# BuTTerK3ks/AA-RMVSNet

Measured on AMD Instinct MI355X. Metric: depth-hypotheses/sec (ref-views x H x W x D / s), higher is better.
Workload: dtype fp32-class split-fp16 (3 products: cells, deconvs, omega conv on f16 MFMA, lo*lo dropped, fp32 accumulate; fp32 elsewhere); 1 GPU; dtu_eval_1600x1184_n7_d512; ref_views_per_gpu=1, views=7, H=1184, W=1600, D=512, global_batch=1, parallelism=ref-view shard x1

## Files before the change

aa-rmvsnet_amd/csrc/convlstm.hip:

```cpp
#include <hip/hip_runtime.h>

#include <cstdlib>
#include <cstring>

#include <algorithm>
#include <type_traits>

#include "device_common.h"

namespace aarmvs {

typedef float floatx16 __attribute__((ext_vector_type(16)));

enum SrcMode : int { SRC_PLAIN = 0, SRC_POOL = 1, SRC_GNRELU = 2 };

struct ChanSrc {
  const float* ptr;
  int nch;
  int mode;
  const double* stats;
  const float* gamma;
  const float* beta;
  const double* part;
  int nblk;
  double* stats_out;
};

__device__ __forceinline__ void gn_table(const ChanSrc& s, float* gn, double* red, int tid, int H, int W) {
  if (!s.part) {
    if (tid < 16) {
      const GnStat st = stat_read(s.stats + (tid >> 3) * kSlots * 2, 8.0 * H * W);
      const float sc = st.rstd * s.gamma[tid];
      gn[tid] = sc;
      gn[16 + tid] = s.beta[tid] - st.mean * sc;
    }
    return;
  }
  if (tid < 256) {
    double acc[4] = {0.0, 0.0, 0.0, 0.0};
    for (int i = tid; i < s.nblk; i += 256)
#pragma unroll
      for (int j = 0; j < 4; ++j) acc[j] += s.part[4 * i + j];
#pragma unroll
    for (int j = 0; j < 4; ++j) red[j * 256 + tid] = acc[j];
  }
  __syncthreads();
  for (int o = 128; o > 0; o >>= 1) {
    if (tid < o)
#pragma unroll
      for (int j = 0; j < 4; ++j) red[j * 256 + tid] += red[j * 256 + tid + o];
    __syncthreads();
  }
  if (tid < 16) {
    const int g = tid >> 3;
    const GnStat st = gn_stat_from(red[2 * g * 256], red[(2 * g + 1) * 256], 8.0 * H * W);
    const float sc = st.rstd * s.gamma[tid];
    gn[tid] = sc;
    gn[16 + tid] = s.beta[tid] - st.mean * sc;
  }
  if (blockIdx.x == 0 && tid < 4) s.stats_out[(tid >> 1) * kSlots * 2 + (tid & 1)] = red[tid * 256];
  __syncthreads();
}

struct CellArgs {
  ChanSrc part[3];
  int nparts;
  float* h_new;
  float* c;
  const float* c_in;
  float* z_out;
  const float* wpk;
  const float* bias;
  const unsigned* xbound;
  int B, H, W;
  int skew;
};

constexpr int kHScaleExp = 12;

__device__ __forceinline__ int guard_exp_of(float bound) {
  if (!(bound > 0.0f)) return 0;
  const int k = ilogbf(bound);
  return k >= 134 ? 120 : (k < -100 ? -114 : k - 14);
}
__device__ __forceinline__ int xguard_exp(const unsigned* xb) {
  return xb ? guard_exp_of(__uint_as_float(*xb)) : -kHScaleExp;
}
__device__ __forceinline__ int gguard_exp(const float* gamma, const float* beta, int H, int W) {
  return guard_exp_of(gn_relu_bound(gamma, beta, 8.0 * H * W));
}

constexpr int kMaxParts = 3;

template <int KIND>
struct CellDef;
#ifndef AARMVS_C3DB
#define AARMVS_C3DB 1
#endif
#ifndef AARMVS_C4DB
#define AARMVS_C4DB 0
#endif
#ifndef AARMVS_C3SKEW
#define AARMVS_C3SKEW 3
#endif
#ifndef AARMVS_C4SKEW
#define AARMVS_C4SKEW 0
#endif
#ifndef AARMVS_C4PIPE
#define AARMVS_C4PIPE 0
#endif
template <>
struct CellDef<0> {
  static constexpr int NP = 2, CH[kMaxParts] = {32, 16, 0};
  static constexpr int MODE[kMaxParts] = {SRC_PLAIN, SRC_PLAIN, SRC_PLAIN};
  static constexpr int HID = 16;
  static constexpr int H3RW = 1, H3WAVES = 8, H3DB = 1, H3PIPE = 1, H3MS = 1;
  static constexpr int MIN_WAVES = 1;
  static constexpr int SKEW = 3;
};
template <>
struct CellDef<1> {
  static constexpr int NP = 2, CH[kMaxParts] = {16, 16, 0};
  static constexpr int MODE[kMaxParts] = {SRC_POOL, SRC_PLAIN, SRC_PLAIN};
  static constexpr int HID = 16;
  static constexpr int H3RW = 1, H3WAVES = 8, H3DB = 1, H3PIPE = 1, H3MS = 1;
  static constexpr int MIN_WAVES = 1;
  static constexpr int SKEW = 2;
};
template <>
struct CellDef<2> : CellDef<1> {};
template <>
struct CellDef<3> {
  static constexpr int NP = 3, CH[kMaxParts] = {16, 16, 16};
  static constexpr int MODE[kMaxParts] = {SRC_GNRELU, SRC_PLAIN, SRC_PLAIN};
  static constexpr int HID = 16;
  static constexpr int H3RW = 1, H3WAVES = 8, H3DB = AARMVS_C3DB, H3PIPE = 1, H3MS = 1;
  static constexpr int MIN_WAVES = 1;
  static constexpr int SKEW = AARMVS_C3SKEW;
};
template <>
struct CellDef<4> {
  static constexpr int NP = 3, CH[kMaxParts] = {16, 16, 8};
  static constexpr int MODE[kMaxParts] = {SRC_GNRELU, SRC_PLAIN, SRC_PLAIN};
  static constexpr int HID = 8;
  static constexpr int H3RW = 1, H3WAVES = 8, H3DB = AARMVS_C4DB, H3PIPE = AARMVS_C4PIPE, H3MS = 1;
  static constexpr int MIN_WAVES = 4;
  static constexpr int SKEW = AARMVS_C4SKEW;
};

typedef _Float16 half8 __attribute__((ext_vector_type(8)));
typedef _Float16 half2_t __attribute__((ext_vector_type(2)));

template <int KIND, int RW_ = CellDef<KIND>::H3RW, int WAVES_ = CellDef<KIND>::H3WAVES, int MS_ = 1>
struct H3Cfg {
  using D = CellDef<KIND>;
  static constexpr int CIN = D::CH[0] + D::CH[1] + D::CH[2];
  static constexpr int NCHK = (CIN + 15) / 16;
  static constexpr int HID = D::HID, MT = HID / 8, COUT = 4 * HID;
  static constexpr int RW = RW_, WAVES = WAVES_, MS = MS_, MTL = MT / MS, RWAVES = WAVES / MS;
  static_assert(MT % MS == 0 && WAVES % MS == 0, "whole m-tiles and rows per wave");
  static constexpr int TH = RW * RWAVES, THREADS = WAVES * 64, TW = 32, W2 = TW + 2, TROWS = TH + 2;
  static constexpr int NPIX = TROWS * W2;
  static constexpr int A_HALVES = NCHK * 9 * MT * 64 * 8;
  static constexpr size_t LDS_BYTES = (size_t)A_HALVES * 2 * 2 + (size_t)NPIX * 32 * 2 + 32 * 4;
  static constexpr int c0(int p) { return p == 0 ? 0 : (p == 1 ? D::CH[0] : D::CH[0] + D::CH[1]); }
  static constexpr int chunk_part(int c) {
    return 16 * c < c0(1) ? 0 : (16 * c < c0(2) || D::NP < 3 ? 1 : 2);
  }
  static constexpr int chunk_lc0(int c) { return 16 * c - c0(chunk_part(c)); }
  static constexpr int chunk_nv(int c) {
    return D::CH[chunk_part(c)] - chunk_lc0(c) < 16 ? D::CH[chunk_part(c)] - chunk_lc0(c) : 16;
  }
  static constexpr bool chunk_paired(int c) { return chunk_nv(c) == 8; }
};

__device__ __forceinline__ int h3_pix(int p, int h) { return p * 32 + ((h ^ ((p >> 3) & 1)) << 4); }

typedef float float2_t __attribute__((ext_vector_type(2)));
__device__ __forceinline__ uint32_t h3_split2(float a, float b, uint32_t& lo_bits) {
  const half2_t hi = __builtin_convertvector((float2_t){a, b}, half2_t);
  const half2_t lo = __builtin_convertvector((float2_t){a - (float)hi[0], b - (float)hi[1]}, half2_t);
  lo_bits = __builtin_bit_cast(uint32_t, lo);
  return __builtin_bit_cast(uint32_t, hi);
}

template <int KIND, int RW, int WAVES, int NTH = 0, bool PAIRSKIP = false, int MS = 1>
struct H3PixStager {
  using C = H3Cfg<KIND, RW, WAVES, MS>;
  using D = typename C::D;
  static constexpr int TH = NTH ? NTH : C::THREADS;
  static constexpr int NITEM = 2 * C::NPIX;
  static constexpr int NI = (NITEM + TH - 1) / TH;
  static_assert(NI <= 32, "item mask holds 32 items");
  float val[NI][8][4];
  uint32_t in_mask;
  float xs = 1.0f;

  template <int CH>
  __device__ __forceinline__ void load(const CellArgs& a, int b, int y0, int x0, int tid) {
    constexpr int P = C::chunk_part(CH), MODE = D::MODE[P], NCH = D::CH[P];
    constexpr int LC0 = C::chunk_lc0(CH), NV = C::chunk_nv(CH);
    static_assert(NV % 8 == 0, "chunks hold whole 8-channel halves");
    const ChanSrc& s = a.part[P];
    const int H = a.H, W = a.W;
    const int Hs = MODE == SRC_POOL ? 2 * H : H, Ws = MODE == SRC_POOL ? 2 * W : W;
    const uint32_t nbytes = (uint32_t)NCH * (uint32_t)Hs * (uint32_t)Ws * 4u;
    const __amdgpu_buffer_rsrc_t r = uniform_rsrc(s.ptr + (size_t)b * NCH * Hs * Ws, nbytes);
    in_mask = 0u;
#pragma unroll
    for (int j = 0; j < NI; ++j) {
      const int e = tid + j * TH;
      const int h = e >= C::NPIX ? 1 : 0, p = e - h * C::NPIX;
      if (PAIRSKIP && C::chunk_paired(CH) && h) continue;
      const int row = p / C::W2, col = p - row * C::W2;
      const int gy = y0 - 1 + row, gx = x0 - 1 + col;
      const bool in = e < NITEM && 8 * h < NV && gy >= 0 && gy < H && gx >= 0 && gx < W;
      if (in) in_mask |= 1u << j;
      const uint32_t pix = MODE == SRC_POOL ? (uint32_t)(2 * gy * Ws + 2 * gx) : (uint32_t)(gy * W + gx);
      const uint32_t ob = (pix * (uint32_t)NCH + (uint32_t)(LC0 + 8 * h)) * 4u;
      constexpr int NW = MODE == SRC_POOL ? 4 : 1;
#pragma unroll
      for (int w = 0; w < NW; ++w) {
        const uint32_t o = in ? ob + (uint32_t)(((w >> 1) * Ws + (w & 1)) * NCH * 4) : nbytes;
        const float4 q0 = ld4(r, o), q1 = ld4(r, in ? o + 16u : nbytes);
        val[j][0][w] = q0.x;
        val[j][1][w] = q0.y;
        val[j][2][w] = q0.z;
        val[j][3][w] = q0.w;
        val[j][4][w] = q1.x;
        val[j][5][w] = q1.y;
        val[j][6][w] = q1.z;
        val[j][7][w] = q1.w;
      }
    }
  }

  template <int CH>
  __device__ __forceinline__ void store(char* hi_plane, char* lo_plane, const float* gn, int tid,
                                        int x0, int W) const {
    constexpr int MODE = D::MODE[C::chunk_part(CH)];
    constexpr int LC0 = C::chunk_lc0(CH);
#pragma unroll
    for (int j = 0; j < NI; ++j) {
      const int e = tid + j * TH;
      if (e < NITEM) {
        const int h = e >= C::NPIX ? 1 : 0, p = e - h * C::NPIX;
        if (PAIRSKIP && C::chunk_paired(CH) && h) continue;
        const bool in = in_mask & (1u << j);
        float v[8];
#pragma unroll
        for (int k = 0; k < 8; ++k) {
          float x;
          constexpr float HS = (float)(1 << kHScaleExp);
          if (MODE == SRC_POOL) {
            x = fmaxf(fmaxf(val[j][k][0], val[j][k][1]), fmaxf(val[j][k][2], val[j][k][3])) * HS;
          } else if (MODE == SRC_GNRELU) {
            const int lc = LC0 + 8 * h + k;
            x = fmaxf(val[j][k][0] * gn[lc] + gn[16 + lc], 0.0f) * xs;
          } else if constexpr (KIND == 0 && C::chunk_part(CH) == 0) {
            x = val[j][k][0] * xs;
          } else {
            x = val[j][k][0] * HS;
          }
          v[k] = in ? x : 0.0f;
        }
        uint32_t hw[4], lw[4];
#pragma unroll
        for (int i = 0; i < 4; ++i) hw[i] = h3_split2(v[2 * i], v[2 * i + 1], lw[i]);
        const int off = h3_pix(p, h);
        *reinterpret_cast<u32x4*>(hi_plane + off) = u32x4{hw[0], hw[1], hw[2], hw[3]};
        *reinterpret_cast<u32x4*>(lo_plane + off) = u32x4{lw[0], lw[1], lw[2], lw[3]};
      }
    }
  }
};

template <class C, int KIND, int CH, bool BAL>
__device__ __forceinline__ void xguard_rescale(floatx16 (&acc)[C::MTL][C::RW], floatx16 (&accn)[C::MTL][C::RW],
                                               float xr) {
  if constexpr ((KIND == 0 || C::D::MODE[0] == SRC_GNRELU) && CH > 0 && C::chunk_part(CH) != 0 &&
                C::chunk_part(CH - 1) == 0) {
#pragma unroll
    for (int m = 0; m < C::MTL; ++m)
#pragma unroll
      for (int r = 0; r < C::RW; ++r) {
        acc[m][r] *= xr;
        if constexpr (BAL) accn[m][r] *= xr;
      }
  }
}

template <class C, int CH, bool PIPE = false, bool BAL = true, int ONCE = 0>
__device__ __forceinline__ void h3_mfma_chunk(floatx16 (&acc)[C::MTL][C::RW], floatx16 (&accn)[C::MTL][C::RW],
                                              const char* wl_hi, const char* wl_lo, const char* in_hi,
                                              const char* in_lo, int wave, int lane, int m0 = 0) {
  constexpr int MT = C::MT, MTL = C::MTL, RW = C::RW;
  const int col = lane & 31, h = lane >> 5;
  if constexpr (C::chunk_paired(CH)) {
    int hv;
    asm volatile("v_mov_b32 %0, %1" : "=v"(hv) : "v"(h));
#pragma unroll
    for (int s = 0; s < 5; ++s) {
      const int tap = min(2 * s + hv, 8);
      half8 bh[RW], bl[RW];
#pragma unroll
      for (int r = 0; r < RW; ++r) {
        const int boff = h3_pix((wave * RW + r + tap / 3) * C::W2 + col + tap % 3, 0);
        bh[r] = *reinterpret_cast<const half8*>(in_hi + boff);
        bl[r] = *reinterpret_cast<const half8*>(in_lo + boff);
      }
#pragma unroll
      for (int m = 0; m < MTL; ++m) {
        const int aoff = ((((CH * 9 + s) * MT + m0 + m) * 64) + lane) * 16;
        const half8 ah = *reinterpret_cast<const half8*>(wl_hi + aoff);
        const half8 al = *reinterpret_cast<const half8*>(wl_lo + aoff);
#pragma unroll
        for (int r = 0; r < RW; ++r) {
          floatx16& d = (BAL && ((s + CH) & 1)) ? accn[m][r] : acc[m][r];
          d = __builtin_amdgcn_mfma_f32_32x32x16_f16(ah, bh[r], d, 0, 0, 0);
          d = __builtin_amdgcn_mfma_f32_32x32x16_f16(ah, bl[r], d, 0, 0, 0);
          d = __builtin_amdgcn_mfma_f32_32x32x16_f16(al, bh[r], d, 0, 0, 0);
        }
      }
    }
  } else if constexpr (PIPE) {
    half8 bh[2][RW], bl[2][RW], ah[2][MTL], al[2][MTL];
    auto fetch = [&](int tap, int s) {
      if ((ONCE & 2) && tap > 0) {
#pragma unroll
        for (int r = 0; r < RW; ++r) bh[s][r] = bh[s ^ 1][r], bl[s][r] = bl[s ^ 1][r];
      } else
#pragma unroll
      for (int r = 0; r < RW; ++r) {
        const int boff = h3_pix((wave * RW + r + tap / 3) * C::W2 + col + tap % 3, h);
        bh[s][r] = *reinterpret_cast<const half8*>(in_hi + boff);
        bl[s][r] = *reinterpret_cast<const half8*>(in_lo + boff);
      }
      if ((ONCE & 1) && tap > 0) {
#pragma unroll
        for (int m = 0; m < MTL; ++m) ah[s][m] = ah[s ^ 1][m], al[s][m] = al[s ^ 1][m];
        return;
      }
#pragma unroll
      for (int m = 0; m < MTL; ++m) {
        const int aoff = ((((CH * 9 + tap) * MT + m0 + m) * 64) + lane) * 16;
        ah[s][m] = *reinterpret_cast<const half8*>(wl_hi + aoff);
        al[s][m] = *reinterpret_cast<const half8*>(wl_lo + aoff);
      }
    };
    fetch(0, 0);
#pragma unroll
    for (int tap = 0; tap < 9; ++tap) {
      const int s = tap & 1;
      if (tap + 1 < 9) fetch(tap + 1, s ^ 1);
      __builtin_amdgcn_sched_barrier(0);
#pragma unroll
      for (int m = 0; m < MTL; ++m)
#pragma unroll
        for (int r = 0; r < RW; ++r) {
          floatx16& d = (BAL && ((tap + CH) & 1)) ? accn[m][r] : acc[m][r];
          d = __builtin_amdgcn_mfma_f32_32x32x16_f16(ah[s][m], bh[s][r], d, 0, 0, 0);
          d = __builtin_amdgcn_mfma_f32_32x32x16_f16(ah[s][m], bl[s][r], d, 0, 0, 0);
          d = __builtin_amdgcn_mfma_f32_32x32x16_f16(al[s][m], bh[s][r], d, 0, 0, 0);
        }
      __builtin_amdgcn_sched_barrier(0);
    }
  } else {
#pragma unroll
    for (int tap = 0; tap < 9; ++tap) {
      half8 bh[RW], bl[RW];
#pragma unroll
      for (int r = 0; r < RW; ++r) {
        const int p = (wave * RW + r + tap / 3) * C::W2 + col + tap % 3;
        const int boff = h3_pix(p, h);
        bh[r] = *reinterpret_cast<const half8*>(in_hi + boff);
        bl[r] = *reinterpret_cast<const half8*>(in_lo + boff);
      }
#pragma unroll
      for (int m = 0; m < MTL; ++m) {
        const int aoff = ((((CH * 9 + tap) * MT + m0 + m) * 64) + lane) * 16;
        const half8 ah = *reinterpret_cast<const half8*>(wl_hi + aoff);
        const half8 al = *reinterpret_cast<const half8*>(wl_lo + aoff);
#pragma unroll
        for (int r = 0; r < RW; ++r) {
          floatx16& d = (BAL && ((tap + CH) & 1)) ? accn[m][r] : acc[m][r];
          d = __builtin_amdgcn_mfma_f32_32x32x16_f16(ah, bh[r], d, 0, 0, 0);
          d = __builtin_amdgcn_mfma_f32_32x32x16_f16(ah, bl[r], d, 0, 0, 0);
          d = __builtin_amdgcn_mfma_f32_32x32x16_f16(al, bh[r], d, 0, 0, 0);
        }
      }
    }
  }
}

template <class C>
__device__ __forceinline__ void cell_c_load(const CellArgs& a, int b, int yw, int x, int hi,
                                            float (&cst)[C::MTL][C::RW][4], int m0 = 0) {
#pragma unroll
  for (int m = 0; m < C::MTL; ++m)
#pragma unroll
    for (int r = 0; r < C::RW; ++r) {
      const int y = yw + r;
      float4 v = make_float4(0.f, 0.f, 0.f, 0.f);
      if (y < a.H && x < a.W)
        v = *reinterpret_cast<const float4*>(
            a.c_in + (((size_t)b * a.H + y) * a.W + x) * C::HID + (m0 + m) * 8 + 4 * hi);
      cst[m][r][0] = v.x;
      cst[m][r][1] = v.y;
      cst[m][r][2] = v.z;
      cst[m][r][3] = v.w;
    }
}

template <class C, int ABL, bool PRECISE>
__device__ __forceinline__ void cell_epilogue(const CellArgs& a, const floatx16 (&acc)[C::MTL][C::RW],
                                              const float (&cst)[C::MTL][C::RW][4], float inv_scale,
                                              int b, int yw, int x, int hi, int m0 = 0) {
  constexpr int HID = C::HID;
#pragma unroll
  for (int r = 0; r < C::RW; ++r) {
    const int y = yw + r;
    if (y < a.H && x < a.W) {
      const size_t pix = ((size_t)b * a.H + y) * a.W + x;
#pragma unroll
      for (int ml = 0; ml < C::MTL; ++ml) {
        const int m = m0 + ml;
        float cn[4], hn[4];
#pragma unroll
        for (int q = 0; q < 4; ++q) {
          const int ch = m * 8 + 4 * hi + q;
          const float gi = fmaf(acc[ml][r][q], inv_scale, a.bias[ch]);
          const float gf = fmaf(acc[ml][r][4 + q], inv_scale, a.bias[HID + ch]);
          const float go = fmaf(acc[ml][r][8 + q], inv_scale, a.bias[2 * HID + ch]);
          const float gg = fmaf(acc[ml][r][12 + q], inv_scale, a.bias[3 * HID + ch]);
          if (ABL & 4) {
            cn[q] = gi + gf;
            hn[q] = go + gg + cst[ml][r][q];
          } else if (PRECISE) {
            cn[q] = precise_sigmoid(gf) * cst[ml][r][q] + precise_sigmoid(gi) * precise_tanh(gg);
            hn[q] = precise_sigmoid(go) * precise_tanh(cn[q]);
          } else {
            cn[q] = fast_sigmoid(gf) * cst[ml][r][q] + fast_sigmoid(gi) * fast_tanh(gg);
            hn[q] = fast_sigmoid(go) * fast_tanh(cn[q]);
          }
        }
        const size_t o = pix * HID + m * 8 + 4 * hi;
        *reinterpret_cast<float4*>(a.c + o) = make_float4(cn[0], cn[1], cn[2], cn[3]);
        *reinterpret_cast<float4*>(a.h_new + o) = make_float4(hn[0], hn[1], hn[2], hn[3]);
        if (a.z_out) {
          const size_t P = (size_t)a.H * a.W;
          float* zo = a.z_out + (size_t)b * 4 * HID * P + ((size_t)(m * 2 + hi) * 4 * P + (size_t)y * a.W + x) * 4;
#pragma unroll
          for (int gt = 0; gt < 4; ++gt) {
            float zz[4];
#pragma unroll
            for (int q = 0; q < 4; ++q) {
              const int ch = m * 8 + 4 * hi + q;
              zz[q] = fmaf(acc[ml][r][4 * gt + q], inv_scale, a.bias[gt * HID + ch]);
            }
            *reinterpret_cast<float4*>(zo + gt * P * 4) = make_float4(zz[0], zz[1], zz[2], zz[3]);
          }
        }
      }
    }
  }
}

template <int KIND, int RW = CellDef<KIND>::H3RW, int WAVES = CellDef<KIND>::H3WAVES, int ABL = 0,
          int PIPE = CellDef<KIND>::H3PIPE, bool PRECISE = false, int MS = 1>
__global__ void __launch_bounds__(WAVES * 64) __attribute__((amdgpu_waves_per_eu(CellDef<KIND>::MIN_WAVES))) lstm_cell_h3_kernel(
    CellArgs a, const float* __restrict__ inv_scale_ptr) {
  using C = H3Cfg<KIND, RW, WAVES, MS>;
  using D = typename C::D;
  constexpr int MT = C::MTL, NCHK = C::NCHK;
  extern __shared__ __attribute__((aligned(16))) char lds_h3[];
  char* wl_hi = lds_h3;
  char* wl_lo = wl_hi + C::A_HALVES * 2;
  char* in_hi = wl_lo + C::A_HALVES * 2;
  char* in_lo = in_hi + C::NPIX * 32;
  float* gn = reinterpret_cast<float*>(in_lo + C::NPIX * 32);

  const int tid = threadIdx.x, lane = tid & 63, wave = tid >> 6;
  const int H = a.H, W = a.W;
  const float inv_scale = ldexpf(*inv_scale_ptr, -kHScaleExp);
  {
    const float4* s = reinterpret_cast<const float4*>(a.wpk);
    float4* d = reinterpret_cast<float4*>(wl_hi);
    constexpr int N4 = C::A_HALVES * 2 * 2 / 16;
#pragma unroll 8
    for (int i = tid; i < N4; i += C::THREADS) d[i] = s[i];
  }
#pragma unroll
  for (int p = 0; p < D::NP; ++p)
    if (D::MODE[p] == SRC_GNRELU) gn_table(a.part[p], gn, reinterpret_cast<double*>(in_hi), tid, H, W);

  const int tiles_x = (W + C::TW - 1) / C::TW, tiles_y = (H + C::TH - 1) / C::TH;
  const int ntiles = a.B * tiles_x * tiles_y;
  auto coords = [&](int tile, int& b, int& y0, int& x0) {
    b = tile / (tiles_x * tiles_y);
    const int rem = tile % (tiles_x * tiles_y);
    y0 = (rem / tiles_x) * C::TH;
    x0 = (rem % tiles_x) * C::TW;
  };
  H3PixStager<KIND, RW, WAVES, 0, !PRECISE, MS> st;
  const int xe = KIND == 0 ? xguard_exp(a.xbound)
                 : D::MODE[0] == SRC_GNRELU ? gguard_exp(a.part[0].gamma, a.part[0].beta, H, W) : 0;
  st.xs = ldexpf(1.0f, -xe);
  const float xr = ldexpf(1.0f, xe + kHScaleExp);
  int tile = blockIdx.x;
  if (tile < ntiles && !(ABL & 2)) {
    int b, y0, x0;
    coords(tile, b, y0, x0);
    st.template load<0>(a, b, y0, x0, tid);
  }
  const int hi = lane >> 5, col = lane & 31;
  const int rwave = wave % C::RWAVES, m0 = (wave / C::RWAVES) * C::MTL;
  for (; tile < ntiles; tile += gridDim.x) {
    int b, y0, x0;
    coords(tile, b, y0, x0);
    const int next = tile + (int)gridDim.x;
    int nb = 0, ny0 = 0, nx0 = 0;
    if (next < ntiles) coords(next, nb, ny0, nx0);
    const int yw = y0 + rwave * RW;
    floatx16 acc[MT][RW], accn[MT][RW];
#pragma unroll
    for (int m = 0; m < MT; ++m)
#pragma unroll
      for (int r = 0; r < RW; ++r)
#pragma unroll
        for (int j = 0; j < 16; ++j) acc[m][r][j] = accn[m][r][j] = 0.0f;
    float cst[MT][RW][4];
    auto chunk = [&](auto CHc) {
      constexpr int CH = decltype(CHc)::value;
      __syncthreads();
      if (!(ABL & 2)) st.template store<CH>(in_hi, in_lo, gn, tid, x0, W);
      __syncthreads();
      if (ABL & 2) {
      } else if (CH + 1 < NCHK) {
        st.template load<(CH + 1 < NCHK ? CH + 1 : 0)>(a, b, y0, x0, tid);
      } else if (next < ntiles) {
        st.template load<0>(a, nb, ny0, nx0, tid);
      }
      if (CH == 0) cell_c_load<C>(a, b, yw, x0 + col, hi, cst, m0);
      xguard_rescale<C, KIND, CH, PRECISE>(acc, accn, xr);
      if (!(ABL & 1)) h3_mfma_chunk<C, CH, PIPE != 0, PRECISE, (ABL >> 3) & 3>(acc, accn, wl_hi, wl_lo, in_hi, in_lo, rwave, lane, m0);
    };
    chunk(std::integral_constant<int, 0>{});
    if constexpr (NCHK > 1) chunk(std::integral_constant<int, 1>{});
    if constexpr (NCHK > 2) chunk(std::integral_constant<int, 2>{});
#pragma unroll
    for (int m = 0; m < MT; ++m)
#pragma unroll
      for (int r = 0; r < RW; ++r)
        if constexpr (PRECISE) acc[m][r] -= accn[m][r];
    cell_epilogue<C, ABL, PRECISE>(a, acc, cst, inv_scale, b, yw, x0 + col, hi, m0);
  }
}

template <int KIND, int RW = CellDef<KIND>::H3RW, int WAVES = CellDef<KIND>::H3WAVES, int ABL = 0,
          int PIPE = CellDef<KIND>::H3PIPE, bool PRECISE = false, int MS = 1>
__global__ void __launch_bounds__(WAVES * 64) __attribute__((amdgpu_waves_per_eu(CellDef<KIND>::MIN_WAVES))) lstm_cell_h3db_kernel(
    CellArgs a, const float* __restrict__ inv_scale_ptr) {
  using C = H3Cfg<KIND, RW, WAVES, MS>;
  using D = typename C::D;
  constexpr int MT = C::MTL, NCHK = C::NCHK;
  constexpr int PB = C::NPIX * 32;
  static_assert(NCHK >= 2, "two or more input chunks");
  extern __shared__ __attribute__((aligned(16))) char lds_h3[];
  char* wl_hi = lds_h3;
  char* wl_lo = wl_hi + C::A_HALVES * 2;
  char* inb = wl_lo + C::A_HALVES * 2;
  float* gn = reinterpret_cast<float*>(inb + 4 * PB);

  const int tid = threadIdx.x, lane = tid & 63, wave = tid >> 6;
  const int H = a.H, W = a.W;
  const float inv_scale = ldexpf(*inv_scale_ptr, -kHScaleExp);
  {
    const float4* s = reinterpret_cast<const float4*>(a.wpk);
    float4* d = reinterpret_cast<float4*>(wl_hi);
    constexpr int N4 = C::A_HALVES * 2 * 2 / 16;
#pragma unroll 8
    for (int i = tid; i < N4; i += C::THREADS) d[i] = s[i];
  }
#pragma unroll
  for (int p = 0; p < D::NP; ++p)
    if (D::MODE[p] == SRC_GNRELU) gn_table(a.part[p], gn, reinterpret_cast<double*>(inb), tid, H, W);
  const int tiles_x = (W + C::TW - 1) / C::TW, tiles_y = (H + C::TH - 1) / C::TH;
  const int ntiles = a.B * tiles_x * tiles_y;
  auto coords = [&](int tile, int& b, int& y0, int& x0) {
    b = tile / (tiles_x * tiles_y);
    const int rem = tile % (tiles_x * tiles_y);
    y0 = (rem / tiles_x) * C::TH;
    x0 = (rem % tiles_x) * C::TW;
  };
  int tile = blockIdx.x;
  if (tile >= ntiles) return;
  H3PixStager<KIND, RW, WAVES, 0, false, MS> st;
  const int xe = KIND == 0 ? xguard_exp(a.xbound)
                 : D::MODE[0] == SRC_GNRELU ? gguard_exp(a.part[0].gamma, a.part[0].beta, H, W) : 0;
  st.xs = ldexpf(1.0f, -xe);
  const float xr = ldexpf(1.0f, xe + kHScaleExp);
  int b, y0, x0;
  coords(tile, b, y0, x0);
  if (!(ABL & 2)) st.template load<0>(a, b, y0, x0, tid);
  __syncthreads();
  if (!(ABL & 2)) {
    st.template store<0>(inb, inb + PB, gn, tid, x0, W);
    st.template load<1>(a, b, y0, x0, tid);
  }
  __syncthreads();
  int par = 0;
  const int hi = lane >> 5, col = lane & 31;
  const int rwave = wave % C::RWAVES, m0 = (wave / C::RWAVES) * C::MTL;
  const bool early = a.skew > 0 && ((wave >> (a.skew - 1)) & 1) != 0;
  for (; tile < ntiles; tile += gridDim.x) {
    coords(tile, b, y0, x0);
    const int next = tile + (int)gridDim.x;
    int nb = 0, ny0 = 0, nx0 = 0;
    if (next < ntiles) coords(next, nb, ny0, nx0);
    const int yw = y0 + rwave * RW;
    const int x = x0 + col;
    floatx16 acc[MT][RW], accn[MT][RW];
    float cst[MT][RW][4];
#pragma unroll
    for (int m = 0; m < MT; ++m)
#pragma unroll
      for (int r = 0; r < RW; ++r)
#pragma unroll
        for (int j = 0; j < 16; ++j) acc[m][r][j] = accn[m][r][j] = 0.0f;
    cell_c_load<C>(a, b, yw, x, hi, cst, m0);
    auto step = [&](auto CHc) {
      constexpr int CH = decltype(CHc)::value;
      constexpr bool F_NEXT = CH + 1 >= NCHK;
      constexpr int F = F_NEXT ? 0 : CH + 1;
      constexpr bool A_NEXT = CH + 2 >= NCHK;
      constexpr int AC = A_NEXT ? CH + 2 - NCHK : CH + 2;
      const char* cur = inb + 2 * par * PB;
      char* oth = inb + 2 * (par ^ 1) * PB;
      auto stage = [&] {
        if (!(ABL & 2)) {
          if (!F_NEXT || next < ntiles) st.template store<F>(oth, oth + PB, gn, tid, 0, W);
          if (!A_NEXT)
            st.template load<AC>(a, b, y0, x0, tid);
          else if (next < ntiles)
            st.template load<AC>(a, nb, ny0, nx0, tid);
        }
      };
      if (early) stage();
      xguard_rescale<C, KIND, CH, PRECISE>(acc, accn, xr);
      if (!(ABL & 1)) h3_mfma_chunk<C, CH, PIPE != 0, PRECISE, (ABL >> 3) & 3>(acc, accn, wl_hi, wl_lo, cur, cur + PB, rwave, lane, m0);
      if (!early) stage();
      if constexpr (CH == NCHK - 1) {
#pragma unroll
        for (int m = 0; m < MT; ++m)
#pragma unroll
          for (int r = 0; r < RW; ++r)
            if constexpr (PRECISE) acc[m][r] -= accn[m][r];
        cell_epilogue<C, ABL, PRECISE>(a, acc, cst, inv_scale, b, yw, x, hi, m0);
      }
      __syncthreads();
      par ^= 1;
    };
    step(std::integral_constant<int, 0>{});
    step(std::integral_constant<int, 1>{});
    if constexpr (NCHK > 2) step(std::integral_constant<int, 2>{});
  }
}

template <int KIND, int RW = CellDef<KIND>::H3RW, int WAVES = CellDef<KIND>::H3WAVES, int ABL = 0,
          int DB = CellDef<KIND>::H3DB, int PIPE = CellDef<KIND>::H3PIPE, bool PRECISE = false,
          int MS = CellDef<KIND>::H3MS>
static hipError_t run_cell_h3_(const CellArgs& a, const float* inv_scale, int cu, int kid,
                               hipStream_t s) {
  using C = H3Cfg<KIND, RW, WAVES, MS>;
  constexpr size_t lds = C::LDS_BYTES + (DB ? (size_t)C::NPIX * 32 * 2 : 0);
  static_assert(lds <= 160 * 1024, "h3 cell tile exceeds LDS");
  const void* fn = DB ? (const void*)lstm_cell_h3db_kernel<KIND, RW, WAVES, ABL, PIPE, PRECISE, MS>
                      : (const void*)lstm_cell_h3_kernel<KIND, RW, WAVES, ABL, PIPE, PRECISE, MS>;
  static bool attr_set[kMaxDevices] = {};
  if (hipError_t e = ensure_dyn_lds(fn, (int)lds, attr_set); e != hipSuccess) return e;
  const int ntiles = a.B * ((a.W + C::TW - 1) / C::TW) * ((a.H + C::TH - 1) / C::TH);
  const int per_cu = std::max(1, (int)((160 * 1024) / lds));
  const int grid = std::max(1, std::min(ntiles, cu * per_cu));
  const char* skew_s = std::getenv("AARMVS_CELL_SKEW");
  const int skew_env = (skew_s && *skew_s) ? std::atoi(skew_s) : -1;
  CellArgs ak = a;
  ak.skew = skew_env >= 0 ? skew_env : CellDef<KIND>::SKEW;
  ProfScope ps(s, kid);
  if (DB)
    hipLaunchKernelGGL((lstm_cell_h3db_kernel<KIND, RW, WAVES, ABL, PIPE, PRECISE, MS>), dim3(grid),
                       dim3(C::THREADS), lds, s, ak, inv_scale);
  else
    hipLaunchKernelGGL((lstm_cell_h3_kernel<KIND, RW, WAVES, ABL, PIPE, PRECISE, MS>), dim3(grid),
                       dim3(C::THREADS), lds, s, ak, inv_scale);
  return hipGetLastError();
}
template <int KIND, int RW = CellDef<KIND>::H3RW, int WAVES = CellDef<KIND>::H3WAVES, int ABL = 0,
          int DB = CellDef<KIND>::H3DB, int PIPE = CellDef<KIND>::H3PIPE, int MS = CellDef<KIND>::H3MS>
static hipError_t run_cell_h3(const CellArgs& a, const float* inv_scale, int cu, int kid,
                              hipStream_t s) {
  return a.z_out ? run_cell_h3_<KIND, RW, WAVES, ABL, DB, PIPE, true, MS>(a, inv_scale, cu, kid, s)
                 : run_cell_h3_<KIND, RW, WAVES, ABL, DB, PIPE, false, MS>(a, inv_scale, cu, kid, s);
}

template <int KIND>
static int cell_shape(const CellArgs&, int) {
  const char* e = std::getenv("AARMVS_CELL_MS");
  return (e && *e) ? std::max(0, std::min(2, std::atoi(e))) : 0;
}
template <int KIND>
static hipError_t run_cell(const CellArgs& a, const float* inv_scale, int cu, int kid, hipStream_t s) {
  using D = CellDef<KIND>;
  if constexpr (D::HID >= 16) {
    const int sh = cell_shape<KIND>(a, cu);
    if (sh == 1) return run_cell_h3<KIND, 1, 8, 0, D::H3DB, D::H3PIPE, 2>(a, inv_scale, cu, kid, s);
    if (sh == 2) return run_cell_h3<KIND, 1, 16, 0, D::H3DB, D::H3PIPE, 2>(a, inv_scale, cu, kid, s);
  }
  return run_cell_h3<KIND>(a, inv_scale, cu, kid, s);
}

constexpr int kDpTH = 8, kDpTW = 32;
template <int ABL = 0>
__global__ void __launch_bounds__(256) deconv_px2_kernel(const float* __restrict__ in,
                                                         const float* __restrict__ w,
                                                         const float* __restrict__ bias, int Hi,
                                                         int Wi, float* __restrict__ out,
                                                         double* __restrict__ gn_part) {
  constexpr int SH = kDpTH + 1, SW = kDpTW + 1;
  __shared__ float tin[16][SH][SW];
  __shared__ float4 wsh[16 * 9 * 4];
  __shared__ float red[4 * 4];
  const int b = blockIdx.z, tid = threadIdx.x;
  const int y0 = blockIdx.y * kDpTH, x0 = blockIdx.x * kDpTW;
  const int hc = tid >> 7, r = tid & 127;
  const int tx = r & 31, tyb = r >> 5;
  const int ix = x0 + tx;
  const int Wo = 2 * Wi;
  const float* ib = in + (size_t)b * 16 * Hi * Wi;
  for (int i = tid; i < SH * SW * 4; i += 256) {
    const int c4 = i & 3, px = i >> 2, yy = px / SW, xx = px - yy * SW;
    const int gy = y0 + yy, gx = x0 + xx;
    float4 q = make_float4(0.f, 0.f, 0.f, 0.f);
    if (!(ABL & 4) && gy < Hi && gx < Wi)
      q = *reinterpret_cast<const float4*>(ib + ((size_t)gy * Wi + gx) * 16 + 4 * c4);
    tin[4 * c4 + 0][yy][xx] = q.x;
    tin[4 * c4 + 1][yy][xx] = q.y;
    tin[4 * c4 + 2][yy][xx] = q.z;
    tin[4 * c4 + 3][yy][xx] = q.w;
  }
  for (int i = tid; i < 16 * 9 * 4; i += 256) wsh[i] = reinterpret_cast<const float4*>(w)[i];
  __syncthreads();
  float o[2][4][8];
#pragma unroll
  for (int p = 0; p < 2; ++p)
#pragma unroll
    for (int q = 0; q < 4; ++q)
#pragma unroll
      for (int c = 0; c < 8; ++c) o[p][q][c] = 0.f;
#pragma unroll 1
  for (int ci = 0; ci < ((ABL & 2) ? 1 : 16); ++ci) {
    float v[2][4];
#pragma unroll
    for (int p = 0; p < 2; ++p) {
      const int ty = tyb + 4 * p;
      v[p][0] = tin[ci][ty][tx];
      v[p][1] = tin[ci][ty][tx + 1];
      v[p][2] = tin[ci][ty + 1][tx];
      v[p][3] = tin[ci][ty + 1][tx + 1];
    }
    const float4* wc = wsh + ci * 9 * 4 + 2 * hc;
#pragma unroll
    for (int c4 = 0; c4 < 2; ++c4) {
      float4 kt[9];
#pragma unroll
      for (int t = 0; t < 9; ++t) kt[t] = wc[t * 4 + c4];
#pragma unroll
      for (int u = 0; u < 4; ++u) {
        const int c = 4 * c4 + u;
        auto k = [&](int tap) {
          const float4 q = kt[tap];
          return u == 0 ? q.x : u == 1 ? q.y : u == 2 ? q.z : q.w;
        };
#pragma unroll
        for (int p = 0; p < 2; ++p) {
          const float v00 = v[p][0], v01 = v[p][1], v10 = v[p][2], v11 = v[p][3];
          o[p][0][c] = fmaf(v00, k(4), o[p][0][c]);
          o[p][1][c] = fmaf(v00, k(5), fmaf(v01, k(3), o[p][1][c]));
          o[p][2][c] = fmaf(v00, k(7), fmaf(v10, k(1), o[p][2][c]));
          o[p][3][c] = fmaf(v00, k(8), fmaf(v01, k(6), fmaf(v10, k(2), fmaf(v11, k(0), o[p][3][c]))));
        }
      }
    }
  }
  float part[4] = {0.f, 0.f, 0.f, 0.f};
  float* ob = out + (size_t)b * 16 * 4 * Hi * Wi;
#pragma unroll
  for (int p = 0; p < 2; ++p) {
    const int iy = y0 + tyb + 4 * p;
    if (iy < Hi && ix < Wi) {
#pragma unroll
      for (int q = 0; q < 4; ++q) {
        float4* d = reinterpret_cast<float4*>(ob + ((size_t)(2 * iy + (q >> 1)) * Wo + 2 * ix + (q & 1)) * 16 + 8 * hc);
#pragma unroll
        for (int c4 = 0; c4 < 2; ++c4) {
          float rr[4];
#pragma unroll
          for (int u = 0; u < 4; ++u) {
            rr[u] = o[p][q][4 * c4 + u] + bias[8 * hc + 4 * c4 + u];
            part[2 * hc] += rr[u];
            part[2 * hc + 1] += rr[u] * rr[u];
          }
          if (!(ABL & 1) || rr[0] == 1234.5f) d[c4] = make_float4(rr[0], rr[1], rr[2], rr[3]);
        }
      }
    }
  }
  block_sum<4>(part, red);
  if (tid == 0) {
    double* pp = gn_part + 4 * (((size_t)b * gridDim.y + blockIdx.y) * gridDim.x + blockIdx.x);
#pragma unroll
    for (int j = 0; j < 4; ++j) pp[j] = part[j];
  }
}

typedef _Float16 dhalf8 __attribute__((ext_vector_type(8)));
template <int ABL = 0>
__global__ void __launch_bounds__(256) __attribute__((amdgpu_waves_per_eu(4))) deconv_mfma_kernel(const float* __restrict__ in,
                                                           const float* __restrict__ wfrag,
                                                           const float* __restrict__ bias, int Hi,
                                                           int Wi, float* __restrict__ out,
                                                           double* __restrict__ gn_part) {
  __shared__ dhalf8 afs[12 * 64];
  __shared__ double red[4 * 4];
  const int b = blockIdx.z, tid = threadIdx.x, lane = tid & 63, wave = tid >> 6;
  const int x0 = blockIdx.x * kDpTW;
  const int n = lane & 31, hh = lane >> 5;
  const int Wo = 2 * Wi;
  const float* ib = in + (size_t)b * 16 * Hi * Wi;
  const dhalf8* af = reinterpret_cast<const dhalf8*>(wfrag);
  for (int i = tid; i < 12 * 64; i += 256) afs[i] = af[i];
  const float inv = wfrag[6 * 2 * 64 * 8 / 2] * (1.0f / 16384.0f);
  const int iy0 = blockIdx.y * kDpTH + wave * 2, ix = x0 + n;
  float4 raw[3][2][2];
#pragma unroll
  for (int r = 0; r < 3; ++r)
#pragma unroll
    for (int c = 0; c < 2; ++c) {
      float4 q0 = make_float4(0.f, 0.f, 0.f, 0.f), q1 = q0;
      if (!(ABL & 4) && iy0 + r < Hi && ix + c < Wi) {
        const float4* sp = reinterpret_cast<const float4*>(ib + ((size_t)(iy0 + r) * Wi + ix + c) * 16 + 8 * hh);
        q0 = sp[0];
        q1 = sp[1];
      }
      raw[r][c][0] = q0;
      raw[r][c][1] = q1;
    }
  __syncthreads();
  auto split = [&](const float4 (&q)[2], dhalf8& bh, dhalf8& bl) {
    const float v[8] = {q[0].x, q[0].y, q[0].z, q[0].w, q[1].x, q[1].y, q[1].z, q[1].w};
#pragma unroll
    for (int j = 0; j < 8; j += 2) {
      uint32_t lo;
      const half2_t hi = __builtin_bit_cast(half2_t, h3_split2(v[j] * 16384.0f, v[j + 1] * 16384.0f, lo));
      const half2_t lw = __builtin_bit_cast(half2_t, lo);
      bh[j] = hi[0];
      bh[j + 1] = hi[1];
      bl[j] = lw[0];
      bl[j + 1] = lw[1];
    }
  };
  double part[4] = {0.0, 0.0, 0.0, 0.0};
  typedef float fx16 __attribute__((ext_vector_type(16)));
#pragma unroll
  for (int rr = 0; rr < 2; ++rr) {
    const int iy = iy0 + rr;
    if (iy < Hi) {
      dhalf8 b00h, b00l, b01h, b01l, b10h, b10l, b11h, b11l;
      split(raw[rr][0], b00h, b00l);
      split(raw[rr][1], b01h, b01l);
      split(raw[rr + 1][0], b10h, b10l);
      split(raw[rr + 1][1], b11h, b11l);
      fx16 a01, a23;
#pragma unroll
      for (int r = 0; r < 16; ++r) a01[r] = a23[r] = 0.f;
      if (!(ABL & 2)) {
        auto mm = [&](fx16 acc, int p, dhalf8 bh, dhalf8 bl) {
          const dhalf8 ah = afs[(p * 2 + 0) * 64 + lane], al = afs[(p * 2 + 1) * 64 + lane];
          acc = __builtin_amdgcn_mfma_f32_32x32x16_f16(ah, bh, acc, 0, 0, 0);
          acc = __builtin_amdgcn_mfma_f32_32x32x16_f16(ah, bl, acc, 0, 0, 0);
          acc = __builtin_amdgcn_mfma_f32_32x32x16_f16(al, bh, acc, 0, 0, 0);
          return acc;
        };
        a01 = mm(a01, 0, b00h, b00l);
        a01 = mm(a01, 1, b01h, b01l);
        a23 = mm(a23, 2, b00h, b00l);
        a23 = mm(a23, 3, b01h, b01l);
        a23 = mm(a23, 4, b10h, b10l);
        a23 = mm(a23, 5, b11h, b11l);
      }
      if (ix < Wi) {
        float* ob = out + (size_t)b * 16 * 4 * Hi * Wi;
#pragma unroll
        for (int g = 0; g < 4; ++g) {
          const int slot = g >> 1, c0 = 4 * hh + 8 * (g & 1), grp = g & 1;
#pragma unroll
          for (int acc_i = 0; acc_i < 2; ++acc_i) {
            const fx16& A = acc_i ? a23 : a01;
            const int oy = 2 * iy + acc_i, ox = 2 * ix + slot;
            float v4[4];
#pragma unroll
            for (int u = 0; u < 4; ++u) {
              v4[u] = fmaf(A[4 * g + u], inv, bias[c0 + u]);
              part[2 * grp] += (double)v4[u];
              part[2 * grp + 1] += (double)v4[u] * v4[u];
            }
            float4* d = reinterpret_cast<float4*>(ob + ((size_t)oy * Wo + ox) * 16 + c0);
            if (!(ABL & 1) || v4[0] == 1234.5f) *d = make_float4(v4[0], v4[1], v4[2], v4[3]);
          }
        }
      }
    }
  }
  block_sum_d_store<4>(part, red, gn_part + 4 * (((size_t)b * gridDim.y + blockIdx.y) * gridDim.x + blockIdx.x));
}

constexpr int kHeadTH = 8, kHeadTW = 32;

__device__ __forceinline__ void wta_select(float cost, float dv, float& max_prob, float& depth,
                                           float& exp_sum) {
#pragma clang fp contract(off)
  const float pr = expf(cost);
  const float mp = max_prob;
  const float f = (mp < pr) ? 1.0f : 0.0f;
  max_prob = __fadd_rn(__fmul_rn(f, pr), __fmul_rn(1.0f - f, mp));
  depth = __fadd_rn(__fmul_rn(f, dv), __fmul_rn(1.0f - f, depth));
  exp_sum = __fadd_rn(exp_sum, pr);
}

__global__ void __launch_bounds__(256) wta_update_kernel(const float* __restrict__ cost,
                                                         const float* __restrict__ depth_d,
                                                         float* __restrict__ max_prob,
                                                         float* __restrict__ depth,
                                                         float* __restrict__ exp_sum, int HW) {
  const int b = blockIdx.y;
  const float dv = depth_d[b];
  for (int p = blockIdx.x * blockDim.x + threadIdx.x; p < HW; p += gridDim.x * blockDim.x) {
    const size_t q = (size_t)b * HW + p;
    float mp = max_prob[q], dp = depth[q], es = exp_sum[q];
    wta_select(cost[q], dv, mp, dp, es);
    max_prob[q] = mp;
    depth[q] = dp;
    exp_sum[q] = es;
  }
}

hipError_t launch_wta_update(const float* cost, const float* depth_d, float* max_prob,
                             float* depth, float* exp_sum, int B, int HW, hipStream_t s) {
  const int blocks = std::max(1, std::min((HW + 255) / 256, 4096));
  ProfScope ps(s, K_HEAD_WTA);
  hipLaunchKernelGGL(wta_update_kernel, dim3(blocks, B), dim3(256), 0, s, cost, depth_d, max_prob,
                     depth, exp_sum, HW);
  return hipGetLastError();
}

__global__ void __launch_bounds__(256) head_wta_kernel(const float* __restrict__ h4,
                                                        const float* __restrict__ w,
                                                        const float* __restrict__ bias, int H,
                                                        int W, const float* __restrict__ dvals,
                                                        int d, int D, float* __restrict__ cost_out,
                                                        int wta, float* __restrict__ max_prob,
                                                        float* __restrict__ exp_sum,
                                                        float* __restrict__ depth,
                                                        double* __restrict__ zero_stats,
                                                        int zero_n) {
#pragma clang fp contract(off)
  constexpr int TW2 = kHeadTW + 2, NPX = (kHeadTH + 2) * TW2;
  __shared__ float4 t[NPX][2];
  if (zero_stats && blockIdx.x == 0 && blockIdx.y == 0)
    for (int i = threadIdx.x; i < zero_n; i += blockDim.x) zero_stats[i] = 0.0;
  const int b = blockIdx.y, HW = H * W;
  const int tiles_x = (W + kHeadTW - 1) / kHeadTW;
  const int y0 = (blockIdx.x / tiles_x) * kHeadTH, x0 = (blockIdx.x % tiles_x) * kHeadTW;
  const float* hb = h4 + (size_t)b * 8 * HW;
  const int ty = threadIdx.x / kHeadTW, tx = threadIdx.x % kHeadTW;
  const int y = y0 + ty, x = x0 + tx;
  const bool own = y < H && x < W;
  const int p = own ? y * W + x : 0;
  const size_t q = (size_t)b * HW + p;
  float mp = 0.f, dp = 0.f, es = 0.f;
  if (wta && own) {
    mp = max_prob[q];
// ... 323 lines not shown
```

Before: 1.194 billion depth-hypotheses/s.

## Defer ConvLSTM cell epilogue into next tile's MFMA chunk steps

Adds a deferred-epilogue mode to the double-buffered h3 cell kernel. Each tile's accumulators are saved and their gate math and stores are spread across the next tile's chunk steps, one m-tile per step, so the epilogue overlaps MFMA work and staging. Bias is cached in LDS, and c-state loads are split per m-tile. The mode is on by default only for cell kind 3. It costs extra registers for the saved accumulators plus a tail epilogue after the loop, and a grid-size env override is also added.

```diff
diff --git a/aa-rmvsnet_amd/csrc/convlstm.hip b/aa-rmvsnet_amd/csrc/convlstm.hip
--- a/aa-rmvsnet_amd/csrc/convlstm.hip
+++ b/aa-rmvsnet_amd/csrc/convlstm.hip
@@ -109,6 +109,18 @@
 #ifndef AARMVS_C4PIPE
 #define AARMVS_C4PIPE 0
 #endif
+#ifndef AARMVS_C0DEFER
+#define AARMVS_C0DEFER 0
+#endif
+#ifndef AARMVS_C1DEFER
+#define AARMVS_C1DEFER 0
+#endif
+#ifndef AARMVS_C2DEFER
+#define AARMVS_C2DEFER 0
+#endif
+#ifndef AARMVS_C3DEFER
+#define AARMVS_C3DEFER 1
+#endif
 template <>
 struct CellDef<0> {
   static constexpr int NP = 2, CH[kMaxParts] = {32, 16, 0};
@@ -117,6 +129,7 @@
   static constexpr int H3RW = 1, H3WAVES = 8, H3DB = 1, H3PIPE = 1, H3MS = 1;
   static constexpr int MIN_WAVES = 1;
   static constexpr int SKEW = 3;
+  static constexpr int H3DEFER = AARMVS_C0DEFER;
 };
 template <>
 struct CellDef<1> {
@@ -126,9 +139,12 @@
   static constexpr int H3RW = 1, H3WAVES = 8, H3DB = 1, H3PIPE = 1, H3MS = 1;
   static constexpr int MIN_WAVES = 1;
   static constexpr int SKEW = 2;
+  static constexpr int H3DEFER = AARMVS_C1DEFER;
 };
 template <>
-struct CellDef<2> : CellDef<1> {};
+struct CellDef<2> : CellDef<1> {
+  static constexpr int H3DEFER = AARMVS_C2DEFER;
+};
 template <>
 struct CellDef<3> {
   static constexpr int NP = 3, CH[kMaxParts] = {16, 16, 16};
@@ -137,6 +153,7 @@
   static constexpr int H3RW = 1, H3WAVES = 8, H3DB = AARMVS_C3DB, H3PIPE = 1, H3MS = 1;
   static constexpr int MIN_WAVES = 1;
   static constexpr int SKEW = AARMVS_C3SKEW;
+  static constexpr int H3DEFER = AARMVS_C3DEFER;
 };
 template <>
 struct CellDef<4> {
@@ -146,6 +163,7 @@
   static constexpr int H3RW = 1, H3WAVES = 8, H3DB = AARMVS_C4DB, H3PIPE = AARMVS_C4PIPE, H3MS = 1;
   static constexpr int MIN_WAVES = 4;
   static constexpr int SKEW = AARMVS_C4SKEW;
+  static constexpr int H3DEFER = 0;
 };
 
 typedef _Float16 half8 __attribute__((ext_vector_type(8)));
@@ -393,11 +411,11 @@
   }
 }
 
-template <class C>
+template <class C, int ML0 = 0, int MLN = C::MTL>
 __device__ __forceinline__ void cell_c_load(const CellArgs& a, int b, int yw, int x, int hi,
                                             float (&cst)[C::MTL][C::RW][4], int m0 = 0) {
 #pragma unroll
-  for (int m = 0; m < C::MTL; ++m)
+  for (int m = ML0; m < ML0 + MLN; ++m)
 #pragma unroll
     for (int r = 0; r < C::RW; ++r) {
       const int y = yw + r;
@@ -412,27 +430,29 @@
     }
 }
 
-template <class C, int ABL, bool PRECISE>
+template <class C, int ABL, bool PRECISE, int ML0 = 0, int MLN = C::MTL>
 __device__ __forceinline__ void cell_epilogue(const CellArgs& a, const floatx16 (&acc)[C::MTL][C::RW],
                                               const float (&cst)[C::MTL][C::RW][4], float inv_scale,
-                                              int b, int yw, int x, int hi, int m0 = 0) {
+                                              int b, int yw, int x, int hi, int m0 = 0,
+                                              const float* lbias = nullptr) {
   constexpr int HID = C::HID;
+  const float* bias = lbias ? lbias : a.bias;
 #pragma unroll
   for (int r = 0; r < C::RW; ++r) {
     const int y = yw + r;
     if (y < a.H && x < a.W) {
       const size_t pix = ((size_t)b * a.H + y) * a.W + x;
 #pragma unroll
-      for (int ml = 0; ml < C::MTL; ++ml) {
+      for (int ml = ML0; ml < ML0 + MLN; ++ml) {
         const int m = m0 + ml;
         float cn[4], hn[4];
 #pragma unroll
         for (int q = 0; q < 4; ++q) {
           const int ch = m * 8 + 4 * hi + q;
-          const float gi = fmaf(acc[ml][r][q], inv_scale, a.bias[ch]);
-          const float gf = fmaf(acc[ml][r][4 + q], inv_scale, a.bias[HID + ch]);
-          const float go = fmaf(acc[ml][r][8 + q], inv_scale, a.bias[2 * HID + ch]);
-          const float gg = fmaf(acc[ml][r][12 + q], inv_scale, a.bias[3 * HID + ch]);
+          const float gi = fmaf(acc[ml][r][q], inv_scale, bias[ch]);
+          const float gf = fmaf(acc[ml][r][4 + q], inv_scale, bias[HID + ch]);
+          const float go = fmaf(acc[ml][r][8 + q], inv_scale, bias[2 * HID + ch]);
+          const float gg = fmaf(acc[ml][r][12 + q], inv_scale, bias[3 * HID + ch]);
           if (ABL & 4) {
             cn[q] = gi + gf;
             hn[q] = go + gg + cst[ml][r][q];
@@ -456,7 +476,7 @@
 #pragma unroll
             for (int q = 0; q < 4; ++q) {
               const int ch = m * 8 + 4 * hi + q;
-              zz[q] = fmaf(acc[ml][r][4 * gt + q], inv_scale, a.bias[gt * HID + ch]);
+              zz[q] = fmaf(acc[ml][r][4 * gt + q], inv_scale, bias[gt * HID + ch]);
             }
             *reinterpret_cast<float4*>(zo + gt * P * 4) = make_float4(zz[0], zz[1], zz[2], zz[3]);
           }
@@ -558,7 +578,7 @@
 }
 
 template <int KIND, int RW = CellDef<KIND>::H3RW, int WAVES = CellDef<KIND>::H3WAVES, int ABL = 0,
-          int PIPE = CellDef<KIND>::H3PIPE, bool PRECISE = false, int MS = 1>
+          int PIPE = CellDef<KIND>::H3PIPE, bool PRECISE = false, int MS = 1, bool DEFER = false>
 __global__ void __launch_bounds__(WAVES * 64) __attribute__((amdgpu_waves_per_eu(CellDef<KIND>::MIN_WAVES))) lstm_cell_h3db_kernel(
     CellArgs a, const float* __restrict__ inv_scale_ptr) {
   using C = H3Cfg<KIND, RW, WAVES, MS>;
@@ -566,11 +586,13 @@
   constexpr int MT = C::MTL, NCHK = C::NCHK;
   constexpr int PB = C::NPIX * 32;
   static_assert(NCHK >= 2, "two or more input chunks");
+  static_assert(!DEFER || (!PRECISE && MT <= NCHK), "deferred: inference, one m-tile per step");
   extern __shared__ __attribute__((aligned(16))) char lds_h3[];
   char* wl_hi = lds_h3;
   char* wl_lo = wl_hi + C::A_HALVES * 2;
   char* inb = wl_lo + C::A_HALVES * 2;
   float* gn = reinterpret_cast<float*>(inb + 4 * PB);
+  float* lbias = gn + 32;
 
   const int tid = threadIdx.x, lane = tid & 63, wave = tid >> 6;
   const int H = a.H, W = a.W;
@@ -582,6 +604,8 @@
 #pragma unroll 8
     for (int i = tid; i < N4; i += C::THREADS) d[i] = s[i];
   }
+  if constexpr (DEFER)
+    if (tid < C::COUT) lbias[tid] = a.bias[tid];
 #pragma unroll
   for (int p = 0; p < D::NP; ++p)
     if (D::MODE[p] == SRC_GNRELU) gn_table(a.part[p], gn, reinterpret_cast<double*>(inb), tid, H, W);
@@ -613,6 +637,10 @@
   const int hi = lane >> 5, col = lane & 31;
   const int rwave = wave % C::RWAVES, m0 = (wave / C::RWAVES) * C::MTL;
   const bool early = a.skew > 0 && ((wave >> (a.skew - 1)) & 1) != 0;
+  floatx16 pacc[MT][RW];
+  int pb = 0, pyw = 0, px = 0;
+  bool pending = false;
+  float cst[MT][RW][4];
   for (; tile < ntiles; tile += gridDim.x) {
     coords(tile, b, y0, x0);
     const int next = tile + (int)gridDim.x;
@@ -621,14 +649,13 @@
     const int yw = y0 + rwave * RW;
     const int x = x0 + col;
     floatx16 acc[MT][RW], accn[MT][RW];
-    float cst[MT][RW][4];
 #pragma unroll
     for (int m = 0; m < MT; ++m)
 #pragma unroll
       for (int r = 0; r < RW; ++r)
 #pragma unroll
         for (int j = 0; j < 16; ++j) acc[m][r][j] = accn[m][r][j] = 0.0f;
-    cell_c_load<C>(a, b, yw, x, hi, cst, m0);
+    if constexpr (!DEFER) cell_c_load<C>(a, b, yw, x, hi, cst, m0);
     auto step = [&](auto CHc) {
       constexpr int CH = decltype(CHc)::value;
       constexpr bool F_NEXT = CH + 1 >= NCHK;
@@ -646,17 +673,41 @@
             st.template load<AC>(a, nb, ny0, nx0, tid);
         }
       };
-      if (early) stage();
+      auto gates = [&] {
+        if constexpr (DEFER && CH < MT) {
+          if (pending) {
+            cell_epilogue<C, ABL, PRECISE, CH, 1>(a, pacc, cst, inv_scale, pb, pyw, px, hi, m0, lbias);
+            if constexpr (CH + 1 < MT) cell_c_load<C, CH + 1, 1>(a, pb, pyw, px, hi, cst, m0);
+          }
+        }
+      };
+      if (early) {
+        gates();
+        stage();
+      }
       xguard_rescale<C, KIND, CH, PRECISE>(acc, accn, xr);
       if (!(ABL & 1)) h3_mfma_chunk<C, CH, PIPE != 0, PRECISE, (ABL >> 3) & 3>(acc, accn, wl_hi, wl_lo, cur, cur + PB, rwave, lane, m0);
-      if (!early) stage();
+      if (!early) {
+        gates();
+        stage();
+      }
       if constexpr (CH == NCHK - 1) {
-#pragma unroll
-        for (int m = 0; m < MT; ++m)
-#pragma unroll
-          for (int r = 0; r < RW; ++r)
-            if constexpr (PRECISE) acc[m][r] -= accn[m][r];
-        cell_epilogue<C, ABL, PRECISE>(a, acc, cst, inv_scale, b, yw, x, hi, m0);
+        if constexpr (DEFER) {
+#pragma unroll
+          for (int m = 0; m < MT; ++m)
+#pragma unroll
+            for (int r = 0; r < RW; ++r) pacc[m][r] = acc[m][r];
+          pb = b, pyw = yw, px = x;
+          pending = true;
+          cell_c_load<C, 0, 1>(a, b, yw, x, hi, cst, m0);
+        } else {
+#pragma unroll
+          for (int m = 0; m < MT; ++m)
+#pragma unroll
+            for (int r = 0; r < RW; ++r)
+              if constexpr (PRECISE) acc[m][r] -= accn[m][r];
+          cell_epilogue<C, ABL, PRECISE>(a, acc, cst, inv_scale, b, yw, x, hi, m0);
+        }
       }
       __syncthreads();
       par ^= 1;
@@ -665,6 +716,10 @@
     step(std::integral_constant<int, 1>{});
     if constexpr (NCHK > 2) step(std::integral_constant<int, 2>{});
   }
+  if constexpr (DEFER) {
+    if constexpr (MT > 1) cell_c_load<C, 1, MT - 1>(a, pb, pyw, px, hi, cst, m0);
+    cell_epilogue<C, ABL, PRECISE>(a, pacc, cst, inv_scale, pb, pyw, px, hi, m0, lbias);
+  }
 }
 
 template <int KIND, int RW = CellDef<KIND>::H3RW, int WAVES = CellDef<KIND>::H3WAVES, int ABL = 0,
@@ -673,20 +728,39 @@
 static hipError_t run_cell_h3_(const CellArgs& a, const float* inv_scale, int cu, int kid,
                                hipStream_t s) {
   using C = H3Cfg<KIND, RW, WAVES, MS>;
-  constexpr size_t lds = C::LDS_BYTES + (DB ? (size_t)C::NPIX * 32 * 2 : 0);
-  static_assert(lds <= 160 * 1024, "h3 cell tile exceeds LDS");
+  constexpr size_t lds_base = C::LDS_BYTES + (DB ? (size_t)C::NPIX * 32 * 2 : 0);
+  static_assert(lds_base + C::COUT * 4 <= 160 * 1024, "h3 cell tile exceeds LDS");
+  constexpr bool HAS_DEFER = DB && !PRECISE && MS == CellDef<KIND>::H3MS &&
+                             RW == CellDef<KIND>::H3RW && WAVES == CellDef<KIND>::H3WAVES;
+  bool defer = false;
+  if constexpr (HAS_DEFER) {
+    const char* defer_s = std::getenv("AARMVS_CELL_DEFER");
+    defer = (defer_s && *defer_s) ? std::atoi(defer_s) != 0 : CellDef<KIND>::H3DEFER != 0;
+  }
+  const size_t lds = lds_base + (defer ? C::COUT * 4 : 0);
   const void* fn = DB ? (const void*)lstm_cell_h3db_kernel<KIND, RW, WAVES, ABL, PIPE, PRECISE, MS>
                       : (const void*)lstm_cell_h3_kernel<KIND, RW, WAVES, ABL, PIPE, PRECISE, MS>;
-  static bool attr_set[kMaxDevices] = {};
-  if (hipError_t e = ensure_dyn_lds(fn, (int)lds, attr_set); e != hipSuccess) return e;
+  if constexpr (HAS_DEFER)
+    if (defer) fn = (const void*)lstm_cell_h3db_kernel<KIND, RW, WAVES, ABL, PIPE, PRECISE, MS, true>;
+  static bool attr_set[2][kMaxDevices] = {};
+  if (hipError_t e = ensure_dyn_lds(fn, (int)lds, attr_set[defer]); e != hipSuccess) return e;
   const int ntiles = a.B * ((a.W + C::TW - 1) / C::TW) * ((a.H + C::TH - 1) / C::TH);
   const int per_cu = std::max(1, (int)((160 * 1024) / lds));
-  const int grid = std::max(1, std::min(ntiles, cu * per_cu));
+  const char* grid_s = std::getenv("AARMVS_CELL_GRID");
+  const int grid_env = (grid_s && *grid_s) ? std::atoi(grid_s) : 0;
+  const int grid = std::max(1, std::min(grid_env > 0 ? grid_env : ntiles, cu * per_cu));
   const char* skew_s = std::getenv("AARMVS_CELL_SKEW");
   const int skew_env = (skew_s && *skew_s) ? std::atoi(skew_s) : -1;
   CellArgs ak = a;
   ak.skew = skew_env >= 0 ? skew_env : CellDef<KIND>::SKEW;
   ProfScope ps(s, kid);
+  if constexpr (HAS_DEFER) {
+    if (defer) {
+      hipLaunchKernelGGL((lstm_cell_h3db_kernel<KIND, RW, WAVES, ABL, PIPE, PRECISE, MS, true>), dim3(grid),
+                         dim3(C::THREADS), lds, s, ak, inv_scale);
+      return hipGetLastError();
+    }
+  }
   if (DB)
     hipLaunchKernelGGL((lstm_cell_h3db_kernel<KIND, RW, WAVES, ABL, PIPE, PRECISE, MS>), dim3(grid),
                        dim3(C::THREADS), lds, s, ak, inv_scale);
```

Result: no change. 1.193 billion depth-hypotheses/s (-0.1%).
